# Kebii/MikuDance

Hardware: AMD Instinct MI355X
Metric: frames/sec (768x768, 16f, 20 DDIM steps) (higher is better)
Workload: dtype f16; 1 GPU; configs[1]: 768x768, 16-frame clip, 20 DDIM steps, fp16, reference_unet + denoising_unet + motion_module, CFG 3.5, one clip per GPU per step; parallelism=dp1, input_staging=rank-local (every rank stages its own clip in HBM before the timed region), reference_reuse=True, queues=1, weights=random-init SD-1.5 geometry (N(0,1/fan_in), seeds 1234/4321), width=full

## Files before the change

### include/mdance_hip.h

```cpp
#ifndef MDANCE_HIP_H
#define MDANCE_HIP_H
#include <stddef.h>
#ifdef __cplusplus
extern "C" {
#endif

#define MD_ACT_NONE 0
#define MD_ACT_SILU 1
#define MD_ACT_RELU 2
#define MD_ACT_GEGLU 3
#define MD_ACT_QUICKGELU 4

int md_version(void);
const char* md_last_error(void);

int md_gemm_f16(const void* A, int lda, const void* W, void* C, int ldc, int M, int N, int K, const void* bias,
                const void* residual, int ldr, const void* rowadd, int ldra, int rows_per_group, int act,
                int transpose_out, void* stream);

int md_conv3x3_nhwc_f16(const void* X, const void* W, void* Y, int ldy, int B, int Hin, int Win, int Cin, int Cout,
                        int stride, int upsample, const void* bias, const void* residual, int ldr,
                        const void* rowadd, int ldra, int rows_per_group, int act, void* stream);

int md_conv3x3_pad_nhwc_f16(const void* X, const void* W, void* Y, int ldy, int B, int Hin, int Win, int Cin, int Cout,
                            int stride, int upsample, int pad_lo, const void* bias, const void* residual, int ldr,
                            const void* rowadd, int ldra, int rows_per_group, int act, void* stream);

int md_conv_nhwc_f16(const void* X, int ldx, const void* W, void* Y, int ldy, int B, int Hin, int Win, int Cin, int Cout, int kw,
                     int stride, int upsample, int pad_lo, const void* bias, const void* residual, int ldr, const void* rowadd,
                     int ldra, int rows_per_group, int act, void* stream);

int md_softmax_rows_f16(void* x, int ldx, int rows, int cols, float scale, void* stream);

size_t md_groupnorm_workspace_bytes(int B, int HW, int C, int G);
int md_groupnorm_nhwc_f16(const void* x, void* y, const void* gamma, const void* beta, int B, int HW, int C, int G,
                          float eps, int silu, void* workspace, size_t ws_bytes, void* stream);

int md_groupnorm_ld_nhwc_f16(const void* x, int ldx, void* y, const void* gamma, const void* beta, int B, int HW, int C, int G,
                             float eps, int silu, void* workspace, size_t ws_bytes, void* stream);

int md_layernorm_f16(const void* x, void* y, void* y2, const void* gamma, const void* beta, const void* add, int M,
                     int C, float eps, int add_mode, int add_row_begin, int rows_per_frame, int frames, void* stream);

int md_groupnorm_plan(int B, int HW, int C, int G, int ldx, int x_align16, int table, int* threads, int* R, int* slab, int* nslab);

int md_layernorm_plan(int M, int C);

int md_gemm_ln_plan(int M, int N, int K, int act, int epi);
int md_gemm_ln_f16(const void* A, int lda, const void* Wf, const float* sc, void* C, int ldc, int M, int N, int K, float eps,
                   const void* rowadd, int ldra, int rows_per_group, int act, void* stream);

int md_groupnorm_table_f16(const void* x, int ldx, const void* gamma, const void* beta, int B, int HW, int C, int G, float eps,
                           float* table, void* workspace, size_t ws_bytes, void* stream);
int md_gemm_affine_plan(int M, int N, int K, int rows_per_image);
int md_gemm_affine_f16(const void* A, int lda, const float* table, int rows_per_image, const void* W, void* C, int ldc, int M, int N,
                       int K, const void* bias, void* stream);

int md_instnorm_spade_f16(const void* x, const void* gamma_beta, void* y, int B, int HW, int C, float eps,
                          void* stream);

int md_instnorm_spade_ld_f16(const void* x, int ldx, const void* gamma_beta, void* y, int B, int HW, int C, float eps,
                             void* stream);

int md_attention_fwd_f16(const void* Q, int ldq, const void* K, int ldk, const void* Vt, int ldvt, void* O, int ldo,
                         const int* kv_index, int B, int H, int D, int Lq, int Lk, int kv_stride, float scale,
                         void* stream);

int md_attention_plan(int D, int Lq, int Lk, int kv_stride, int ldvt, int vt_align16);

int md_temporal_attention_fwd_f16(const void* Q, int ldq, const void* K, int ldk, const void* V, int ldv, void* O,
                                  int ldo, int NB, int F, int HW, int H, int D, float scale, void* stream);

int md_temporal_attention_plan(int NB, int F, int HW, int H, int D, int aligned16, int* hg, int* pb);

int md_pack_nhwc_f16(const void* src, int src_is_f32, void* dst, int N, int F, long sB, long sF, long sC, long sY,
                     long sX, int c_begin, int c_count, int Cpad, int Ho, int Wo, int Hin, int Win, void* stream);
int md_unpack_nhwc_f16(const void* src, int ldc, void* dst, int dst_is_f32, int N, int F, long sB, long sF, long sC,
                       long sY, long sX, int C, int Ho, int Wo, void* stream);

int md_concat_channels_f16(const void* a, int Ca, const void* b, int Cb, void* out, long M, void* stream);

int md_window_accumulate(const void* pred, void* noise_sum, void* counter, const int* window, int f, int Ftot, int HW,
                         int halves, void* stream);
// ... 76 lines not shown
```

### mikudance_amd/_lib.py

```python
import ctypes
import os
from ctypes import c_char_p, c_float, c_int, c_long, c_size_t, c_void_p

_HERE = os.path.dirname(os.path.abspath(__file__))
LIB_PATH = os.path.join(_HERE, "libmdance_hip.so")

P = c_void_p
SIGNATURES = {
    "md_version": (c_int, []),
    "md_last_error": (c_char_p, []),
    "md_gemm_f16": (c_int, [P, c_int, P, P, c_int, c_int, c_int, c_int, P, P, c_int, P, c_int, c_int, c_int, c_int, P]),
    "md_conv3x3_nhwc_f16": (c_int, [P, P, P, c_int, c_int, c_int, c_int, c_int, c_int, c_int, c_int, P, P, c_int, P, c_int,
                                    c_int, c_int, P]),
    "md_conv3x3_pad_nhwc_f16": (c_int, [P, P, P, c_int, c_int, c_int, c_int, c_int, c_int, c_int, c_int, c_int, P, P, c_int, P,
                                        c_int, c_int, c_int, P]),
    "md_conv_nhwc_f16": (c_int, [P, c_int, P, P, c_int, c_int, c_int, c_int, c_int, c_int, c_int, c_int, c_int, c_int, P, P, c_int, P,
                                 c_int, c_int, c_int, P]),
    "md_set_cu_limit": (c_int, [c_int]),
    "md_gemm_plan": (c_int, [c_int, c_int, c_int, c_int, c_int, c_int, c_int]),
    "md_conv3x3_plan": (c_int, [c_int, c_int, c_int, c_int, c_int, c_int, c_int, c_int, c_int]),
    "md_gemm_plan_call": (c_int, [P, c_int, P, P, c_int, c_int, c_int, c_int, P, P, c_int, P, c_int, c_int, c_int, c_int,
                                  ctypes.POINTER(c_int), ctypes.POINTER(c_int)]),
    "md_conv_plan_call": (c_int, [P, c_int, P, P, c_int, c_int, c_int, c_int, c_int, c_int, c_int, c_int, c_int, c_int, P, P, c_int, P,
                                  c_int, c_int, c_int]),
    "md_softmax_rows_f16": (c_int, [P, c_int, c_int, c_int, c_float, P]),
    "md_groupnorm_workspace_bytes": (c_size_t, [c_int, c_int, c_int, c_int]),
    "md_groupnorm_nhwc_f16": (c_int, [P, P, P, P, c_int, c_int, c_int, c_int, c_float, c_int, P, c_size_t, P]),
    "md_groupnorm_ld_nhwc_f16": (c_int, [P, c_int, P, P, P, c_int, c_int, c_int, c_int, c_float, c_int, P, c_size_t, P]),
    "md_instnorm_spade_ld_f16": (c_int, [P, c_int, P, P, c_int, c_int, c_int, c_float, P]),
    "md_layernorm_f16": (c_int, [P, P, P, P, P, P, c_int, c_int, c_float, c_int, c_int, c_int, c_int, P]),
    "md_groupnorm_plan": (c_int, [c_int, c_int, c_int, c_int, c_int, c_int, c_int] + [ctypes.POINTER(c_int)] * 4),
    "md_layernorm_plan": (c_int, [c_int, c_int]),
    "md_gemm_ln_plan": (c_int, [c_int, c_int, c_int, c_int, c_int]),
    "md_gemm_ln_f16": (c_int, [P, c_int, P, P, P, c_int, c_int, c_int, c_int, c_float, P, c_int, c_int, c_int, P]),
    "md_groupnorm_table_f16": (c_int, [P, c_int, P, P, c_int, c_int, c_int, c_int, c_float, P, P, c_size_t, P]),
    "md_gemm_affine_plan": (c_int, [c_int, c_int, c_int, c_int]),
    "md_gemm_affine_f16": (c_int, [P, c_int, P, c_int, P, P, c_int, c_int, c_int, c_int, P, P]),
    "md_instnorm_spade_f16": (c_int, [P, P, P, c_int, c_int, c_int, c_float, P]),
    "md_attention_fwd_f16": (c_int, [P, c_int, P, c_int, P, c_int, P, c_int, P, c_int, c_int, c_int, c_int, c_int, c_int,
                                     c_float, P]),
    "md_attention_plan": (c_int, [c_int, c_int, c_int, c_int, c_int, c_int]),
    "md_temporal_attention_fwd_f16": (c_int, [P, c_int, P, c_int, P, c_int, P, c_int, c_int, c_int, c_int, c_int, c_int,
                                              c_float, P]),
    "md_temporal_attention_plan": (c_int, [c_int, c_int, c_int, c_int, c_int, c_int, ctypes.POINTER(c_int), ctypes.POINTER(c_int)]),
    "md_pack_nhwc_f16": (c_int, [P, c_int, P, c_int, c_int, c_long, c_long, c_long, c_long, c_long, c_int, c_int, c_int,
                                 c_int, c_int, c_int, c_int, P]),
    "md_unpack_nhwc_f16": (c_int, [P, c_int, P, c_int, c_int, c_int, c_long, c_long, c_long, c_long, c_long, c_int, c_int,
                                   c_int, P]),
    "md_concat_channels_f16": (c_int, [P, c_int, P, c_int, P, c_long, P]),
    "md_window_accumulate": (c_int, [P, P, P, P, c_int, c_int, c_int, c_int, P]),
    "md_window_accumulate_weighted": (c_int, [P, P, P, P, P, c_int, c_int, c_int, c_int, P]),
    "md_cfg_ddim_step": (c_int, [P, P, P, c_int, c_int, c_int, c_float, c_float, c_float, P]),
    "md_cfg_ddim_step_eta": (c_int, [P, P, P, P, c_int, c_int, c_int, c_float, c_float, c_float, c_float, P]),
    "md_cfg_multistep_step": (c_int, [P, P, P, P, P, c_int, c_int, c_int, c_float, c_float, c_float, c_float, c_float, c_float, c_float, P]),
    "md_cfg_rescale_workspace_bytes": (c_size_t, [c_int, c_int]),
    "md_cfg_guidance_rescale": (c_int, [P, P, c_int, c_int, c_int, c_float, c_float, P, c_size_t, P, P]),
    "md_cfg_ddim_step_scaled": (c_int, [P, P, P, P, P, c_int, c_int, c_int, c_float, c_float, c_float, c_float, P]),
    "md_cfg_multistep_step_scaled": (c_int, [P, P, P, P, P, P, c_int, c_int, c_int, c_float, c_float, c_float, c_float, c_float, c_float,
                                             c_float, P]),
    "md_cfg_apg_workspace_bytes": (c_size_t, [c_int, c_int]),
    "md_cfg_apg_prepare": (c_int, [P, P, P, P, c_int, c_int, c_int, c_float, c_float, c_float, c_float, c_float, P, c_size_t, P, P]),
    "md_cfg_ddim_step_apg": (c_int, [P, P, P, P, P, P, c_int, c_int, c_int, c_float, c_float, c_float, c_float, P]),
    "md_cfg_multistep_step_apg": (c_int, [P, P, P, P, P, P, P, c_int, c_int, c_int, c_float, c_float, c_float, c_float, c_float, c_float,
                                          c_float, P]),
    "md_cfg_ddim_step_pag": (c_int, [P, P, P, P, P, c_int, c_int, c_int, c_float, c_float, c_float, c_float, c_float, P]),
    "md_cfg_multistep_step_pag": (c_int, [P, P, P, P, P, P, c_int, c_int, c_int, c_float, c_float, c_float, c_float, c_float, c_float, c_float,
                                          c_float, P]),
# ... 76 lines not shown
```

### mikudance_amd/blocks.py

```python
from dataclasses import dataclass

import torch
from torch import nn

from . import ops, packing

GROUPS = 32
HEADS = 8


class _Packed(nn.Module):

    def __init__(self):
        super().__init__()
        self._pk = None

    def _apply(self, fn, *a, **k):
        self._pk = None
        return super()._apply(fn, *a, **k)

    def _load_from_state_dict(self, *a, **k):
        self._pk = None
        return super()._load_from_state_dict(*a, **k)

# ... 101 lines not shown
    def __init__(self, dim, kv_dim=None):
        super().__init__()
        self.to_q = Linear(dim, dim, bias=False)
        self.to_k = Linear(kv_dim or dim, dim, bias=False)
        self.to_v = Linear(kv_dim or dim, dim, bias=False)
        self.to_out = nn.ModuleList([Linear(dim, dim)])


class _GEGLU(nn.Module):
    def __init__(self, dim):
        super().__init__()
        self.proj = Linear(dim, dim * 8)


class FeedForward(nn.Module):

    def __init__(self, dim):
        super().__init__()
        self.net = nn.ModuleList([_GEGLU(dim), nn.Identity(), Linear(dim * 4, dim)])


def _pack_ff(ff, dev, pk, prefix="ff"):
    w, b = packing.geglu_weight(ff.net[0].proj.weight, ff.net[0].proj.bias, dev)
    pk[prefix + "1"], pk[prefix + "1b"] = w, b
    pk[prefix + "2"], pk[prefix + "2b"] = packing.linear_weight(ff.net[2].weight, dev), packing.vec(ff.net[2].bias, dev)


FUSE_NORMS = __import__("os").environ.get("MD_FUSE_NORMS", "1") != "0"


def ln_linear(pk, h, norm, lin, bias=None, rowadd=None, rows_per_group=0, act=ops.ACT_NONE, eps=1e-5):
    M, K = h.shape
    w = pk[lin]
    if FUSE_NORMS and ops.gemm_ln_plan(M, w.shape[0], K, act, rowadd is not None, a=h):
        fk = lin + ":ln"
        if fk not in pk:
            pk[fk] = packing.ln_fold(w, None if bias is None else pk[bias], pk[norm + "w"], pk[norm + "b"])
        wf, sc = pk[fk]
        return ops.gemm_ln(h, wf, sc, eps=eps, rowadd=rowadd, rows_per_group=rows_per_group, act=act)
    n = ops.layernorm(h, pk[norm + "w"], pk[norm + "b"], eps=eps)
    return ops.gemm(n, w, bias=None if bias is None else pk[bias], rowadd=rowadd, rows_per_group=rows_per_group, act=act)


def gn_linear(x, gamma, beta, eps, w, bias):
    B, C = x.shape[0], x.shape[-1]
    M = x.numel() // C
    if FUSE_NORMS and ops.gemm_affine_plan(M, w.shape[0], C, M // B, x=x):
        return ops.gemm_affine(x, ops.groupnorm_table(x, gamma, beta, GROUPS, eps), w, bias=bias)
    return ops.gemm(tokens(ops.groupnorm(x, gamma, beta, GROUPS, eps)), w, bias=bias)


def _run_ff(pk, h, norm, prefix="ff"):
    g = ln_linear(pk, h, norm, prefix + "1", bias=prefix + "1b", act=ops.ACT_GEGLU)
    return ops.gemm(g, pk[prefix + "2"], bias=pk[prefix + "2b"], residual=h)


class CrossContext:

    def __init__(self, ctx, index, lk, lpad, zero_frames=0):
        self.ctx, self.index, self.lk, self.lpad = ctx, index, lk, lpad
        self.zero_frames = zero_frames
        self.root = self
        self._slices = {}

    def rows(self, lo, hi):
        s = self._slices.get((lo, hi))
        if s is None:
            s = CrossContext(self.ctx, self.index[lo:hi].contiguous(), self.lk, self.lpad, zero_frames=max(0, min(self.zero_frames, hi) - lo))
            s.root = self.root
            self._slices[(lo, hi)] = s
        return s
# ... 290 lines not shown
```

### mikudance_amd/csrc/gemm.hip

```cpp
#include "common.h"
#include <stdlib.h>
#include <algorithm>


enum { ACT_NONE = 0, ACT_SILU = 1, ACT_RELU = 2, ACT_GEGLU = 3, ACT_QUICKGELU = 4 };

struct GemmParams {
  const half_t* A;
  const half_t* W;
  half_t* C;
  const half_t* bias;
  const half_t* residual;
  const half_t* rowadd;
  int lda, ldc, ldr, ldra;
  int M, N, K;
  int rows_per_group;
  int act;
  int transpose_out;
  int bias_rows;
  int Hin, Win, Cin, Hout, Wout, stride, upsample, pad;
  int ldx;
  int kw;
  int tiles_n, tiles_total;
  int tiles_m, group_m;
  int reverse;
};

__device__ __attribute__((aligned(64))) half_t g_zero_page[32] = {};

typedef const __attribute__((address_space(1))) void* gptr_t;
typedef __attribute__((address_space(3))) void* lptr_t;

template <int N>
__device__ __forceinline__ void wait_vmcnt() {
  asm volatile("s_waitcnt vmcnt(%0)" ::"n"(N) : "memory");
}

typedef float float2_t __attribute__((ext_vector_type(2)));
#ifdef MD_DEGRADE_GELU_TANH
__device__ __forceinline__ float md_gelu_tanh(float x) {
  const float u = 0.7978845608f * (x + 0.044715f * x * x * x);
  return 0.5f * x * (1.f + (1.f - 2.f / (__expf(2.f * u) + 1.f)));
}
#endif
__device__ __forceinline__ float2_t gelu_fast2(float2_t x) {
#ifdef MD_DEGRADE_GELU_TANH
  return float2_t{md_gelu_tanh(x.x), md_gelu_tanh(x.y)};
#endif
  const float2_t ax = {__builtin_fabsf(x.x), __builtin_fabsf(x.y)};
  float2_t p = float2_t{5.621299664e-06f, 5.621299664e-06f};
  p = p * ax + float2_t{5.105520901e-05f, 5.105520901e-05f};
  p = p * ax + float2_t{3.968613701e-05f, 3.968613701e-05f};
  p = p * ax + float2_t{3.422739239e-03f, 3.422739239e-03f};
  p = p * ax + float2_t{2.207699846e-02f, 2.207699846e-02f};
  p = p * ax + float2_t{5.207516304e-02f, 5.207516304e-02f};
  p = p * ax + float2_t{1.044273782e+00f, 1.044273782e+00f};
  p = p * p;
  p = p * p;
// ... 846 lines not shown
  plan_operands(p, epi);
  p.ldc = Cout; p.ldr = Cout; p.ldra = Cout; p.lda = Cin;
  p.Hin = Hin; p.Win = Win; p.Cin = Cin; p.stride = stride; p.upsample = upsample; p.pad = 1; p.ldx = Cin; p.kw = 3;
  p.Hout = ((Hin << upsample) + 2 - 3) / stride + 1;
  p.Wout = ((Win << upsample) + 2 - 3) / stride + 1;
  p.M = B * p.Hout * p.Wout; p.N = Cout; p.K = 9 * Cin; p.rows_per_group = p.Hout * p.Wout; p.act = ACT_NONE;
  return gemm_choose(p, true, 2, 0, ncu).k.code;
}

static int plan_call_result(const GemmParams& p, bool conv, int* blocks, int* tail_code) {
  GemmPlan plan;
  const int rc = gemm_plan_checked(p, conv, &plan);
  if (rc != MD_OK) return rc;
  if (blocks) *blocks = plan.blocks;
  if (tail_code) *tail_code = plan.tail.code;
  return plan.k.code;
}

extern "C" int md_gemm_plan_call(const void* A, int lda, const void* W, void* C, int ldc, int M, int N, int K, const void* bias, const void* residual,
                                 int ldr, const void* rowadd, int ldra, int rows_per_group, int act, int transpose_out, int* blocks,
                                 int* tail_code) {
  return plan_call_result(gemm_params(A, lda, W, C, ldc, M, N, K, bias, residual, ldr, rowadd, ldra, rows_per_group, act, transpose_out), false,
                          blocks, tail_code);
}

extern "C" int md_conv_plan_call(const void* X, int ldx, const void* W, void* Y, int ldy, int B, int Hin, int Win, int Cin, int Cout, int kw, int stride,
                                 int upsample, int pad_lo, const void* bias, const void* residual, int ldr, const void* rowadd, int ldra,
                                 int rows_per_group, int act) {
  GemmParams p;
  const int rc = conv_params(&p, X, ldx, W, Y, ldy, B, Hin, Win, Cin, Cout, kw, stride, upsample, pad_lo, bias, residual, ldr, rowadd, ldra,
                             rows_per_group, act);
  return rc != MD_OK ? rc : plan_call_result(p, true, nullptr, nullptr);
}
```

### mikudance_amd/csrc/gemm_sp.h

```cpp
#pragma once
#ifndef SP_ABL
#define SP_ABL 0
#endif

#ifdef SP_TRACE
#define SP_TRACE_N 48
__device__ unsigned long long g_sp_trace[4][SP_TRACE_N][5];
#define SP_STAMP(S)                                                                                           \
  if (!GEGLU && blockIdx.x == 0 && tr_kt < SP_TRACE_N && lane == 0)                                           \
    *reinterpret_cast<unsigned long long*>(smem + (3 * BM + 2 * BN) * 128 + ((wave * SP_TRACE_N + tr_kt) * 5 + (S)) * 8) = __builtin_readcyclecounter();
#else
#define SP_STAMP(S)
#endif

typedef unsigned uint4_t __attribute__((ext_vector_type(4)));

__device__ __attribute__((aligned(64))) half_t g_zero_cols[16384] = {};
__device__ __attribute__((aligned(64))) half_t g_sp_dump[64 * 8];

__device__ __forceinline__ float sp_acc(const floatx16& a, int r) {
  float x;
  asm volatile("v_accvgpr_read_b32 %0, %1" : "=v"(x) : "a"(a[r]));
  return x;
}

template <int MT, int NT, bool RES, bool RA>
struct SpColumn {
  half4_t b[4];
  uint4 r[RES ? MT : 1][2];
  half4_t a[RA ? MT : 1][4];
};

#ifndef SP_EPI_LA
#define SP_EPI_LA 1
#endif
template <int MT, int NT, bool CONV>
constexpr int sp_residual_lookahead() {
  constexpr int la = SP_EPI_LA < NT - 1 ? SP_EPI_LA : NT - 1;
  return CONV && MT * NT >= 15 && la > 1 ? 1 : la;
}

template <int MT, int NT, bool RES, bool RA, bool AGPR = true, bool RB = false, bool CONV = false>
__device__ __forceinline__ void sp_plain_epilogue(const GemmParams& p, const floatx16 (&acc)[MT][NT], int mw, int nw, int lc, int hi) {
  constexpr bool RA_AHEAD = RA && !RES;
  constexpr int LA = RES ? sp_residual_lookahead<MT, NT, CONV>() : 1;
  const half_t* bias = (p.bias && !RB ? p.bias : g_zero_cols) + (RB ? 0 : nw + 4 * hi);
  float rowb[MT];
  bool row_ok[MT];
  const half_t* rrow[MT];
  const half_t* arow[MT];
  half_t* crow[MT][2];
  bool crow_ok[MT][2];
#pragma unroll
  for (int i = 0; i < MT; ++i) {
    const int m = mw + i * 32 + lc;
    row_ok[i] = m < p.M;
    const int mc = row_ok[i] ? m : p.M - 1;
    rowb[i] = RB && p.bias ? (float)p.bias[mc] : 0.f;
    rrow[i] = RES ? p.residual + (size_t)mc * p.ldr + nw + 8 * hi : nullptr;
    arow[i] = RA ? p.rowadd + (size_t)(mc / p.rows_per_group) * p.ldra + nw + 4 * hi : nullptr;
#pragma unroll
    for (int h = 0; h < 2; ++h) {
      const int mr = mw + i * 32 + 16 * h + (lc & 15);
      crow_ok[i][h] = mr < p.M;
      crow[i][h] = p.C + (size_t)(crow_ok[i][h] ? mr : p.M - 1) * p.ldc + nw + 16 * ((lc >> 4) & 1) + 8 * hi;
    }
  }
  half_t* const dump = g_sp_dump + ((lc + 32 * hi) << 3);
  SpColumn<MT, NT, RES, RA> col[LA + 1];
  auto request = [&](SpColumn<MT, NT, RES, RA>& d, int j, bool ahead) {
    if constexpr (!RB) {
#pragma unroll
      for (int gi = 0; gi < 4; ++gi) d.b[gi] = *reinterpret_cast<const half4_t*>(bias + j * 32 + 8 * gi);
    }
    if constexpr (RES) {
#pragma unroll
      for (int i = 0; i < MT; ++i)
#pragma unroll
        for (int pr = 0; pr < 2; ++pr) d.r[i][pr] = *reinterpret_cast<const uint4*>(rrow[i] + j * 32 + 16 * pr);
    }
    if constexpr (RA) {
      if (ahead == RA_AHEAD) {
#pragma unroll
        for (int i = 0; i < MT; ++i)
#pragma unroll
          for (int gi = 0; gi < 4; ++gi) d.a[i][gi] = *reinterpret_cast<const half4_t*>(arow[i] + j * 32 + 8 * gi);
      }
    }
  };
#pragma unroll
  for (int j = 0; j < LA && j < NT; ++j) request(col[j % (LA + 1)], j, true);
#pragma unroll
  for (int j = 0; j < NT; ++j) {
    SpColumn<MT, NT, RES, RA>& c = col[j % (LA + 1)];
    if (j + LA < NT) request(col[(j + LA) % (LA + 1)], j + LA, true);
    if constexpr (RA && !RA_AHEAD) {
#pragma unroll
      for (int i = 0; i < MT; ++i)
#pragma unroll
        for (int gi = 0; gi < 4; ++gi) c.a[i][gi] = *reinterpret_cast<const half4_t*>(arow[i] + j * 32 + 8 * gi);
    }
    __builtin_amdgcn_sched_barrier(0);
    float bf[4][4];
#pragma unroll
    for (int gi = 0; gi < 4; ++gi)
#pragma unroll
      for (int e = 0; e < 4; ++e) bf[gi][e] = RB ? 0.f : (float)c.b[gi][e];
#pragma unroll
    for (int i = 0; i < MT; ++i) {
      unsigned rp[4][2];
      if constexpr (RES) {
#pragma unroll
        for (int pr = 0; pr < 2; ++pr) {
          const uint4 r4 = c.r[i][pr];
          const auto s0 = __builtin_amdgcn_permlane32_swap(r4.x, r4.z, false, false);
          const auto s1 = __builtin_amdgcn_permlane32_swap(r4.y, r4.w, false, false);
          rp[2 * pr][0] = s0[0]; rp[2 * pr][1] = s1[0];
          rp[2 * pr + 1][0] = s0[1]; rp[2 * pr + 1][1] = s1[1];
        }
      }
      unsigned w[4][2];
#pragma unroll
      for (int gi = 0; gi < 4; ++gi) {
        float v[4];
#pragma unroll
        for (int e = 0; e < 4; ++e) {
          v[e] = (AGPR ? sp_acc(acc[i][j], 4 * gi + e) : acc[i][j][4 * gi + e]) + (RB ? rowb[i] : bf[gi][e]);
          if constexpr (RA) v[e] += (float)c.a[i][gi][e];
        }
        if constexpr (RES) {
          half4_t rv;
          __builtin_memcpy(&rv, rp[gi], 8);
#pragma unroll
          for (int e = 0; e < 4; ++e) v[e] += (float)rv[e];
        }
        const half4_t o = {(half_t)v[0], (half_t)v[1], (half_t)v[2], (half_t)v[3]};
        __builtin_memcpy(w[gi], &o, 8);
      }
      unsigned pc[2][4];
#pragma unroll
      for (int pr = 0; pr < 2; ++pr) {
        const auto s0 = __builtin_amdgcn_permlane32_swap(w[2 * pr][0], w[2 * pr + 1][0], false, false);
        const auto s1 = __builtin_amdgcn_permlane32_swap(w[2 * pr][1], w[2 * pr + 1][1], false, false);
        pc[pr][0] = s0[0]; pc[pr][1] = s1[0]; pc[pr][2] = s0[1]; pc[pr][3] = s1[1];
      }
      unsigned lo[4], hi4[4];
#pragma unroll
      for (int d = 0; d < 4; ++d) {
        const auto t = __builtin_amdgcn_permlane16_swap(pc[0][d], pc[1][d], false, false);
        lo[d] = t[0]; hi4[d] = t[1];
      }
#pragma unroll
      for (int h = 0; h < 2; ++h) {
        const uint4 v4 = h ? uint4{hi4[0], hi4[1], hi4[2], hi4[3]} : uint4{lo[0], lo[1], lo[2], lo[3]};
        if (SP_ABL & 64) asm volatile("" ::"v"(v4.x), "v"(v4.y), "v"(v4.z), "v"(v4.w));
        else *reinterpret_cast<uint4*>(crow_ok[i][h] ? crow[i][h] + j * 32 : dump) = v4;
      }
      __builtin_amdgcn_sched_barrier(0);
    }
  }
}

template <bool CONV, bool GEGLU, int MT, int NT, bool RESM = false>
__global__ __launch_bounds__(256, 1) void gemm_sp_kernel(GemmParams p) {
#if defined(__HIP_DEVICE_COMPILE__)
  constexpr int BK = 64;
  constexpr int BM = 64 * MT, BN = 64 * NT;
  constexpr int ROWB = BK * 2, RPI = 1024 / ROWB;
  constexpr int PA = BM / RPI / 4, PB = BN / RPI / 4;
  static_assert(PA + PB == 16 || PA + PB == 14 || PA + PB == 12 || PA + PB == 10, "issue schedule");
  constexpr int NP0 = PA + PB == 10 ? 3 : (PA + PB == 12 ? 4 : 6), NP1 = PA + PB == 10 ? 3 : 4, NP2 = (PA + PB - NP0 - NP1) / 2, NP3 = NP2;
  static_assert(NP0 + NP1 + NP2 + NP3 == PA + PB && PB >= NP0, "issue schedule");
  static_assert(!GEGLU || NT % 2 == 0, "GEGLU pairs 32-column sub-tiles (2q, 2q+1) of a wave");
  constexpr int ASZ = BM * ROWB, WSZ = BN * ROWB, WBASE = 3 * ASZ;
  extern __shared__ __attribute__((aligned(16))) char smem[];

  const int tid = threadIdx.x;
  const int lane = tid & 63;
  const int wave = __builtin_amdgcn_readfirstlane(tid >> 6);
  const int wm = wave >> 1, wn = wave & 1;
  const int lrow = lane >> 3, pslot = lane & 7;
  const int nk = p.K / BK;
  const int nwg = p.tiles_total;
  const int ntile = (nwg - (int)blockIdx.x + (int)gridDim.x - 1) / (int)gridDim.x;

  auto tile_origin = [&](int i, int& m0, int& n0) {
    const int v = (int)blockIdx.x + i * (int)gridDim.x;
    const int q = nwg >> 3, r = nwg & 7, xcd = v & 7, idx = v >> 3;
    int t = (xcd < r ? xcd * (q + 1) : r * (q + 1) + (xcd - r) * q) + idx;
    if (p.reverse) t = nwg - 1 - t;
    const int gsz = p.group_m * p.tiles_n;
    const int grp = t / gsz, first = grp * p.group_m;
    const int rows = min(p.group_m, p.tiles_m - first);
    const int l = t - grp * gsz;
    const int tn = l / rows;
    m0 = (first + l - tn * rows) * BM;
    n0 = tn * BN;
// ... 293 lines not shown
            gelu_fast2_x<8>(gl);
            __builtin_amdgcn_sched_barrier(0);
            unsigned w[4][2];
#pragma unroll
            for (int c = 0; c < 8; ++c) {
              const float2_t hv = (float2_t{sp_acc(acc[i][2 * q], 2 * c), sp_acc(acc[i][2 * q], 2 * c + 1)} + bh[c]) * gl[c];
              typedef _Float16 h2_t __attribute__((ext_vector_type(2)));
              const h2_t o = {(half_t)hv.x, (half_t)hv.y};
              __builtin_memcpy(&w[c >> 1][c & 1], &o, 4);
            }
            unsigned pc[2][4];
#pragma unroll
            for (int pr = 0; pr < 2; ++pr) {
              const auto s0 = __builtin_amdgcn_permlane32_swap(w[2 * pr][0], w[2 * pr + 1][0], false, false);
              const auto s1 = __builtin_amdgcn_permlane32_swap(w[2 * pr][1], w[2 * pr + 1][1], false, false);
              pc[pr][0] = s0[0]; pc[pr][1] = s1[0]; pc[pr][2] = s0[1]; pc[pr][3] = s1[1];
            }
            uint4 vv[2];
            {
              const auto t0 = __builtin_amdgcn_permlane16_swap(pc[0][0], pc[1][0], false, false);
              const auto t1 = __builtin_amdgcn_permlane16_swap(pc[0][1], pc[1][1], false, false);
              const auto t2 = __builtin_amdgcn_permlane16_swap(pc[0][2], pc[1][2], false, false);
              const auto t3 = __builtin_amdgcn_permlane16_swap(pc[0][3], pc[1][3], false, false);
              vv[0] = uint4{t0[0], t1[0], t2[0], t3[0]};
              vv[1] = uint4{t0[1], t1[1], t2[1], t3[1]};
            }
#pragma unroll
            for (int h = 0; h < 2; ++h) *reinterpret_cast<uint4*>(drow[h]) = vv[h];
            __builtin_amdgcn_sched_barrier(0);
          }
        }
      } else {
        const int mw = m0 + wm * (32 * MT), nw = n0 + wn * (32 * NT);
        if constexpr (RESM) {
          if (p.rowadd) sp_plain_epilogue<MT, NT, false, true>(p, acc, mw, nw, lc, hi);
          else sp_plain_epilogue<MT, NT, false, false>(p, acc, mw, nw, lc, hi);
        } else if (p.bias_rows) sp_plain_epilogue<MT, NT, false, false, true, true>(p, acc, mw, nw, lc, hi);
        else if (p.residual && p.rowadd && !(SP_ABL & 32)) sp_plain_epilogue<MT, NT, true, true, true, false, CONV>(p, acc, mw, nw, lc, hi);
        else if (p.residual && !(SP_ABL & 32)) sp_plain_epilogue<MT, NT, true, false, true, false, CONV>(p, acc, mw, nw, lc, hi);
        else if (p.rowadd) sp_plain_epilogue<MT, NT, false, true>(p, acc, mw, nw, lc, hi);
        else sp_plain_epilogue<MT, NT, false, false>(p, acc, mw, nw, lc, hi);
      }
    }
  }
  wait_vmcnt<0>();
#ifdef SP_TRACE
  if (!GEGLU && blockIdx.x == 0) {
    __syncthreads();
    for (int i = tid; i < 4 * SP_TRACE_N * 5; i += 256)
      (&g_sp_trace[0][0][0])[i] = *reinterpret_cast<const unsigned long long*>(smem + (3 * BM + 2 * BN) * 128 + i * 8);
  }
#endif
#undef SP_TRACE_NEXT
#undef SP_BODY
#undef SP_STEP
#undef SP_RES_MULT
#undef SP_RES_ISSUE
#endif
}

template <bool CONV, bool GEGLU, int NT>
static bool sp_eligible(const GemmParams& p) {
  constexpr int BN = 64 * NT;
  if (p.transpose_out || p.N % BN != 0 || p.K % 64 != 0 || p.K < 128 || (p.N > 16384 && !p.bias_rows)) return false;
  if (p.bias_rows && (p.residual || p.rowadd || CONV || GEGLU)) return false;
  if (!GEGLU && p.act != ACT_NONE) return false;
  if (CONV && p.Cin % 64 != 0) return false;
// ... 3 lines not shown
  if (!al16(p.C) || p.ldc % 8 != 0) return false;
  if (p.bias && !p.bias_rows && !al16(p.bias)) return false;
  if (p.residual && (!al16(p.residual) || p.ldr % 8 != 0)) return false;
  if (p.rowadd && (!al16(p.rowadd) || p.ldra % 8 != 0)) return false;
  return true;
}

template <int MT, int NT>
static bool sp_resm(const GemmParams& p) {
  static const int resm = md_env_int("MD_SP_RESM", 1);
  return resm && p.residual && !p.bias_rows && !(SP_ABL & 32) && p.K / 64 >= MT * NT + 1 &&
         ((unsigned long long)(p.M - 1) * p.ldr + p.N) * 2 < (1ull << 31);
}

template <bool CONV, bool GEGLU, int NT, int MT>
static void launch_sp(GemmParams& p, bool resm, int ncu, hipStream_t stream) {
  constexpr int BM = 64 * MT, BN = 64 * NT;
#ifdef SP_TRACE
  constexpr size_t smem = (size_t)(3 * BM + 2 * BN) * 128 + (GEGLU ? 0 : 4 * SP_TRACE_N * 5 * 8);
  static_assert(smem <= 160 * 1024, "trace build: the stamps live behind the ring");
#else
  constexpr size_t smem = (size_t)(3 * BM + 2 * BN) * 128;
#endif
  md_ensure_dynamic_lds<gemm_sp_kernel<CONV, GEGLU, MT, NT>>((int)smem);
  constexpr int group_m = 8;
  p.tiles_n = p.N / BN;
  p.tiles_m = cdiv(p.M, BM);
  p.tiles_total = p.tiles_m * p.tiles_n;
  p.group_m = group_m;
  static const int rev = md_env_int("MD_SP_REVERSE", 1);
  const bool big_a = (size_t)p.M * (size_t)p.lda * 2 > ((size_t)256 << 20);
  p.reverse = !CONV && !GEGLU && !p.bias_rows && big_a && (rev == 2 || (rev == 1 && p.K >= 4 * p.N));
  const int grid = p.tiles_total < ncu ? p.tiles_total : ncu;
  if constexpr (!GEGLU) {
    if (resm) {
      md_ensure_dynamic_lds<gemm_sp_kernel<CONV, false, MT, NT, true>>((int)smem);
      hipLaunchKernelGGL((gemm_sp_kernel<CONV, false, MT, NT, true>), dim3(grid), dim3(256), smem, stream, p);
      return;
    }
  }
  hipLaunchKernelGGL((gemm_sp_kernel<CONV, GEGLU, MT, NT>), dim3(grid), dim3(256), smem, stream, p);
}

#ifdef SP_TRACE
extern "C" int md_debug_sp_trace(void* dst) {
  return (int)hipMemcpyFromSymbol(dst, HIP_SYMBOL(g_sp_trace), sizeof(unsigned long long) * 4 * SP_TRACE_N * 5);
}
#endif
```

### mikudance_amd/csrc/norm.hip

```cpp
#include "common.h"
#ifndef GN_UNROLL
#define GN_UNROLL 4
#endif
#ifndef GN_THREADS
#define GN_THREADS 512
#endif
template <typename T>
__device__ __forceinline__ void norm_store(T* p, const T& v) { *p = v; }
#ifndef GN_SLAB
#define GN_SLAB 32
#endif

__device__ __forceinline__ float med3(float a, float b, float c) { return fmaxf(fminf(a, b), fminf(fmaxf(a, b), c)); }
__device__ __forceinline__ float gn_pilot(const half_t* __restrict__ ximg, int HW, int ldx, int g, int cpg) {
  const half_t* p = ximg + g * cpg;
  return med3((float)p[0], (float)p[(size_t)(HW >> 1) * ldx + (cpg >> 1)], (float)p[(size_t)(HW - 1) * ldx + cpg - 1]);
}
__global__ void gn_stats_kernel(const half_t* __restrict__ x, float* __restrict__ part, float* __restrict__ pilot, int HW, int C, int ldx, int G, int R,
                                int slab, int nslab) {
  extern __shared__ float sh[];
  const int cch = C >> 3;
  const int cc = threadIdx.x % cch, r = threadIdx.x / cch;
  const int b = blockIdx.y, sl = blockIdx.x;
  const int p0 = sl * slab, p1 = min(p0 + slab, HW);
// ... 573 lines not shown
  if (C == 320) return 720;
#endif
  return 700 + (C <= 512 ? 1 : C <= 1024 ? 2 : C <= 1536 ? 3 : 4);
}

extern "C" int md_layernorm_plan(int M, int C) { return ln_plan(M, C); }

extern "C" int md_layernorm_f16(const void* x, void* y, void* y2, const void* gamma, const void* beta, const void* add, int M, int C, float eps,
                                int add_mode, int add_row_begin, int rows_per_frame, int frames, void* stream) {
  const int code = ln_plan(M, C);
  if (code < 0) return code;
  MD_CHECK_ARG(add_mode == 0 || (add != nullptr && y2 != nullptr), "md_layernorm: add_mode needs add and y2");
  MD_CHECK_ARG(add_mode != 2 || (rows_per_frame > 0 && frames > 0), "md_layernorm: add_mode 2 needs rows_per_frame and frames");
  const dim3 grid(cdiv(M, 4 * LN_R)), block(256);
  hipStream_t st = (hipStream_t)stream;
  if (code == 720) {
    hipLaunchKernelGGL(layernorm320_kernel, dim3(cdiv(M, 32)), block, 0, st, (const half_t*)x, (half_t*)y, (half_t*)y2, (const half_t*)gamma,
                       (const half_t*)beta, (const half_t*)add, M, eps, add_mode, add_row_begin, rows_per_frame, frames);
    MD_CHECK_LAUNCH("md_layernorm");
    return MD_OK;
  }
#define LN_LAUNCH(MC)                                                                                                                          \
  hipLaunchKernelGGL(layernorm_kernel<MC>, grid, block, 0, st, (const half_t*)x, (half_t*)y, (half_t*)y2, (const half_t*)gamma, (const half_t*)beta, \
                     (const half_t*)add, M, C, eps, add_mode, add_row_begin, rows_per_frame, frames)
  if (code == 701) LN_LAUNCH(1);
  else if (code == 702) LN_LAUNCH(2);
  else if (code == 703) LN_LAUNCH(3);
  else LN_LAUNCH(4);
#undef LN_LAUNCH
  MD_CHECK_LAUNCH("md_layernorm");
  return MD_OK;
}

__global__ __launch_bounds__(256) void instnorm_spade_kernel(const half_t* __restrict__ x, const half_t* __restrict__ gb, half_t* __restrict__ y, int HW,
                                                             int C, int ldx, float eps) {
  __shared__ float ss[32][64], sq[32][64], mean_s[64], rstd_s[64];
  const int cc = threadIdx.x & 7, r = threadIdx.x >> 3;
  const int b = blockIdx.y, c0 = blockIdx.x * 64 + cc * 8;
  const half_t* xb = x + (size_t)b * HW * ldx + c0;
  const half8_t ka = *reinterpret_cast<const half8_t*>(xb), kb = *reinterpret_cast<const half8_t*>(xb + (size_t)(HW >> 1) * ldx),
                kc = *reinterpret_cast<const half8_t*>(xb + (size_t)(HW - 1) * ldx);
  float k8[8];
#pragma unroll
  for (int e = 0; e < 8; ++e) k8[e] = med3((float)ka[e], (float)kb[e], (float)kc[e]);
  float s[8], q[8];
#pragma unroll
  for (int e = 0; e < 8; ++e) s[e] = q[e] = 0.f;
  for (int p = r; p < HW; p += 32) {
    const half8_t v = *reinterpret_cast<const half8_t*>(xb + (size_t)p * ldx);
#pragma unroll
    for (int e = 0; e < 8; ++e) {
      const float f = (float)v[e] - k8[e];
      s[e] += f;
      q[e] += f * f;
    }
  }
#pragma unroll
  for (int e = 0; e < 8; ++e) {
    ss[r][cc * 8 + e] = s[e];
    sq[r][cc * 8 + e] = q[e];
  }
  __syncthreads();
  if (threadIdx.x < 64) {
    float a = 0.f, c2 = 0.f;
    for (int rr = 0; rr < 32; ++rr) {
      a += ss[rr][threadIdx.x];
// ... 81 lines not shown
```

### mikudance_amd/ops.py

```python
import ctypes

import torch

from . import _lib

ACT_NONE, ACT_SILU, ACT_RELU, ACT_GEGLU, ACT_QUICKGELU = 0, 1, 2, 3, 4
F16 = torch.float16


def _st():
    return torch.cuda.current_stream().cuda_stream


def _p(t):
    return 0 if t is None else t.data_ptr()


def _chk(t, name, dtype=F16):
    if t is None:
        return
    if not t.is_cuda:
        raise _lib.MdanceHipError(f"{name} must live on the GPU: mikudance_amd has no CPU path")
    if t.dtype != dtype:
        raise _lib.MdanceHipError(f"{name} must be {dtype}, got {t.dtype}")
# ... 92 lines not shown
                    2.0 * B * Ho * Wo * cout * 3 * kw * Cin, 2.0 * (B * H * W * Cin + cout * 3 * kw * Cin + B * Ho * Wo * cout)))
    return out


def conv_plan(x, w, cout, bias=None, residual=None, rowadd=None, rows_per_group=0, act=ACT_NONE, stride=1, upsample=False,
              out=None, pad_lo=1, kw=3):
    args, _, _ = _conv_args(x, w, cout, bias, residual, rowadd, rows_per_group, act, stride, upsample, out, pad_lo, kw)
    return _lib.load().md_conv_plan_call(*args)


def _dense16(t):
    return t is None or (t.data_ptr() % 16 == 0 and t.stride(-2) % 8 == 0 and t.stride(-1) == 1)


def gemm_ln_plan(M, N, K, act=ACT_NONE, rowadd=False, a=None):
    return _dense16(a) and bool(_lib.load().md_gemm_ln_plan(M, N, K, act, 2 if rowadd else 0))


def gemm_ln(a, wf, sc, eps=1e-5, rowadd=None, rows_per_group=0, act=ACT_NONE, out=None):
    lda = _rowmajor(a, "a")
    _chk(wf, "wf"); _chk(sc, "sc", torch.float32); _chk(rowadd, "rowadd")
    M, K = a.shape
    N = wf.shape[0]
    assert wf.shape[1] == K and wf.is_contiguous() and sc.shape == (2, N) and sc.is_contiguous(), (wf.shape, sc.shape, K)
    if out is None:
        out = torch.empty((M, N // 2 if act == ACT_GEGLU else N), device=a.device, dtype=F16)
    ldc = _rowmajor(out, "out")
    ldra = _rowmajor(rowadd, "rowadd") if rowadd is not None else 0
    if rowadd is not None and (rows_per_group <= 0 or rowadd.shape[0] * rows_per_group < M or rowadd.shape[1] < N):
        raise _lib.MdanceHipError(f"gemm_ln: row term {tuple(rowadd.shape)} does not cover M={M} rows in groups of {rows_per_group} x N={N}")
    _lib.call("md_gemm_ln_f16", a.data_ptr(), lda, wf.data_ptr(), sc.data_ptr(), out.data_ptr(), ldc, M, N, K, float(eps), _p(rowadd), ldra,
              rows_per_group, act, _st(),
              meta=(f"gemm M={M} N={N} K={K}" + (" geglu" if act == ACT_GEGLU else "") + " ln", 2.0 * M * N * K, 2.0 * (M * K + N * K + M * N)))
    return out


_workspaces = {}


def _workspace(who, device, need, dtype=torch.float32, floor=0):
    cache = _workspaces.setdefault(who, {})
    key = (device, torch.cuda.current_stream().cuda_stream)
    ws = cache.get(key)
    if ws is None or ws.numel() * dtype.itemsize < need:
        ws = cache[key] = torch.empty((max(need, floor) + dtype.itemsize - 1) // dtype.itemsize, device=device, dtype=dtype)
    return ws


def _gn_workspace(x, B, HW, C, groups):
    return _workspace("groupnorm", x.device, _lib.load().md_groupnorm_workspace_bytes(B, HW, C, groups), floor=1 << 20)


def gemm_affine_plan(M, N, K, rows_per_image, x=None):
    return _dense16(x) and bool(_lib.load().md_gemm_affine_plan(M, N, K, rows_per_image))


def groupnorm_table(x, gamma, beta, groups, eps):
    _chk(gamma, "gamma"); _chk(beta, "beta")
    ldx = _pixel_pitch(x, "x")
    B, C = x.shape[0], x.shape[-1]
    HW = x.numel() // (B * C)
    ws = _gn_workspace(x, B, HW, C, groups)
    table = torch.empty((B, 2, C), device=x.device, dtype=torch.float32)
    _lib.call("md_groupnorm_table_f16", x.data_ptr(), ldx, gamma.data_ptr(), beta.data_ptr(), B, HW, C, groups, float(eps), table.data_ptr(),
              ws.data_ptr(), ws.numel() * 4, _st(), meta=(f"groupnorm B={B} HW={HW} C={C} stats", 0.0, 2.0 * B * HW * C))
    return table
# ... 379 lines not shown
```

Baseline: 7.351 frames/s.

## Fold LayerNorm into GEMM epilogue via precomputed row stats kernel

After: 7.368 frames/s, median of 3. Within noise of the previous version (+0.2%).

```diff
diff --git a/include/mdance_hip.h b/include/mdance_hip.h
--- a/include/mdance_hip.h
+++ b/include/mdance_hip.h
@@ -49,6 +49,12 @@
 int md_gemm_ln_plan(int M, int N, int K, int act, int epi);
 int md_gemm_ln_f16(const void* A, int lda, const void* Wf, const float* sc, void* C, int ldc, int M, int N, int K, float eps,
                    const void* rowadd, int ldra, int rows_per_group, int act, void* stream);
+
+int md_row_stats_plan(int M, int C, int ldx, int x_align16);
+int md_row_stats_f16(const void* x, int ldx, float* stats, int M, int C, float eps, void* stream);
+int md_gemm_ln_stats_plan(int M, int N, int K, int act, int epi);
+int md_gemm_ln_stats_f16(const void* A, int lda, const void* Wf, const float* sc, const float* stats, void* C, int ldc, int M, int N,
+                         int K, const void* rowadd, int ldra, int rows_per_group, int act, void* stream);
 
 int md_groupnorm_table_f16(const void* x, int ldx, const void* gamma, const void* beta, int B, int HW, int C, int G, float eps,
                            float* table, void* workspace, size_t ws_bytes, void* stream);
diff --git a/mikudance_amd/_lib.py b/mikudance_amd/_lib.py
--- a/mikudance_amd/_lib.py
+++ b/mikudance_amd/_lib.py
@@ -33,6 +33,10 @@
     "md_layernorm_plan": (c_int, [c_int, c_int]),
     "md_gemm_ln_plan": (c_int, [c_int, c_int, c_int, c_int, c_int]),
     "md_gemm_ln_f16": (c_int, [P, c_int, P, P, P, c_int, c_int, c_int, c_int, c_float, P, c_int, c_int, c_int, P]),
+    "md_row_stats_plan": (c_int, [c_int, c_int, c_int, c_int]),
+    "md_row_stats_f16": (c_int, [P, c_int, P, c_int, c_int, c_float, P]),
+    "md_gemm_ln_stats_plan": (c_int, [c_int, c_int, c_int, c_int, c_int]),
+    "md_gemm_ln_stats_f16": (c_int, [P, c_int, P, P, P, P, c_int, c_int, c_int, c_int, P, c_int, c_int, c_int, P]),
     "md_groupnorm_table_f16": (c_int, [P, c_int, P, P, c_int, c_int, c_int, c_int, c_float, P, P, c_size_t, P]),
     "md_gemm_affine_plan": (c_int, [c_int, c_int, c_int, c_int]),
     "md_gemm_affine_f16": (c_int, [P, c_int, P, c_int, P, P, c_int, c_int, c_int, c_int, P, P]),
diff --git a/mikudance_amd/blocks.py b/mikudance_amd/blocks.py
--- a/mikudance_amd/blocks.py
+++ b/mikudance_amd/blocks.py
@@ -157,11 +157,15 @@
 def ln_linear(pk, h, norm, lin, bias=None, rowadd=None, rows_per_group=0, act=ops.ACT_NONE, eps=1e-5):
     M, K = h.shape
     w = pk[lin]
-    if FUSE_NORMS and ops.gemm_ln_plan(M, w.shape[0], K, act, rowadd is not None, a=h):
+    fused = FUSE_NORMS and ops.gemm_ln_plan(M, w.shape[0], K, act, rowadd is not None, a=h)
+    swept = FUSE_NORMS and not fused and ops.gemm_ln_stats_plan(M, w.shape[0], K, act, rowadd is not None, a=h)
+    if fused or swept:
         fk = lin + ":ln"
         if fk not in pk:
             pk[fk] = packing.ln_fold(w, None if bias is None else pk[bias], pk[norm + "w"], pk[norm + "b"])
         wf, sc = pk[fk]
+        if swept:
+            return ops.gemm_ln_stats(h, wf, sc, ops.row_stats(h, eps=eps), rowadd=rowadd, rows_per_group=rows_per_group, act=act)
         return ops.gemm_ln(h, wf, sc, eps=eps, rowadd=rowadd, rows_per_group=rows_per_group, act=act)
     n = ops.layernorm(h, pk[norm + "w"], pk[norm + "b"], eps=eps)
     return ops.gemm(n, w, bias=None if bias is None else pk[bias], rowadd=rowadd, rows_per_group=rows_per_group, act=act)
diff --git a/mikudance_amd/csrc/gemm.hip b/mikudance_amd/csrc/gemm.hip
--- a/mikudance_amd/csrc/gemm.hip
+++ b/mikudance_amd/csrc/gemm.hip
@@ -24,6 +24,8 @@
   int tiles_n, tiles_total;
   int tiles_m, group_m;
   int reverse;
+  const float* lnst;
+  const float* lnsc;
 };
 
 __device__ __attribute__((aligned(64))) half_t g_zero_page[32] = {};
@@ -936,3 +938,40 @@
                              rows_per_group, act);
   return rc != MD_OK ? rc : plan_call_result(p, true, nullptr, nullptr);
 }
+
+static int ln_stats_classes() {
+  static const int m = md_env_int("MD_LN_STATS", 3);
+  return m;
+}
+
+static int ln_stats_code(const GemmPlan& plan, const GemmParams& p) {
+  if (p.act != ACT_NONE || p.residual || p.transpose_out || p.K < 640) return 0;
+  if (plan.blocks != 1 || !plan.k.tile || plan.k.swapped || plan.k.resm) return 0;
+  return 3000 + plan.k.tile->code;
+}
+
+extern "C" int md_gemm_ln_stats_plan(int M, int N, int K, int act, int epi) {
+  if (M <= 0 || N <= 0 || K <= 0 || K % 64 || (epi & 1)) return 0;
+  if (!(ln_stats_classes() & ((epi & 2) ? 2 : 1))) return 0;
+  GemmParams p = {};
+  plan_operands(p, epi & 2);
+  p.M = M; p.N = N; p.K = K; p.lda = K; p.ldc = N; p.ldra = N; p.rows_per_group = M; p.act = act;
+  int sp, force_nt;
+  gemm_knobs(&sp, &force_nt);
+  return ln_stats_code(gemm_choose(p, false, sp, force_nt, md_device_cus()), p);
+}
+
+extern "C" int md_gemm_ln_stats_f16(const void* A, int lda, const void* Wf, const float* sc, const float* stats, void* C, int ldc, int M, int N, int K,
+                                    const void* rowadd, int ldra, int rows_per_group, int act, void* stream) {
+  GemmParams p = gemm_params(A, lda, Wf, C, ldc, M, N, K, nullptr, nullptr, 0, rowadd, ldra, rows_per_group, act, 0);
+  GemmPlan plan;
+  if (const int rc = gemm_plan_checked(p, false, &plan)) return rc;
+  MD_CHECK_ARG(ln_stats_code(plan, p) != 0, "md_gemm_ln_stats: no row-affine kernel for M=%d N=%d K=%d act=%d (ask md_gemm_ln_stats_plan first)", M, N, K, act);
+  MD_CHECK_ARG(sc != nullptr && al16(sc) && stats != nullptr && (reinterpret_cast<uintptr_t>(stats) & 7) == 0,
+               "md_gemm_ln_stats: sc must be 16-byte aligned, stats 8-byte aligned");
+  MD_CHECK_ARG((const void*)stats != C && A != C, "md_gemm_ln_stats: in place is not supported");
+  p.lnst = stats; p.lnsc = sc;
+  gemm_launch(plan, p, (hipStream_t)stream);
+  MD_CHECK_LAUNCH("md_gemm_ln_stats");
+  return MD_OK;
+}
diff --git a/mikudance_amd/csrc/gemm_sp.h b/mikudance_amd/csrc/gemm_sp.h
--- a/mikudance_amd/csrc/gemm_sp.h
+++ b/mikudance_amd/csrc/gemm_sp.h
@@ -24,9 +24,10 @@
   return x;
 }
 
-template <int MT, int NT, bool RES, bool RA>
+template <int MT, int NT, bool RES, bool RA, bool LNS = false>
 struct SpColumn {
   half4_t b[4];
+  floatx4 s[LNS ? 4 : 1], c[LNS ? 4 : 1];
   uint4 r[RES ? MT : 1][2];
   half4_t a[RA ? MT : 1][4];
 };
@@ -40,11 +41,14 @@
   return CONV && MT * NT >= 15 && la > 1 ? 1 : la;
 }
 
-template <int MT, int NT, bool RES, bool RA, bool AGPR = true, bool RB = false, bool CONV = false>
+template <int MT, int NT, bool RES, bool RA, bool AGPR = true, bool RB = false, bool CONV = false, bool LNS = false>
 __device__ __forceinline__ void sp_plain_epilogue(const GemmParams& p, const floatx16 (&acc)[MT][NT], int mw, int nw, int lc, int hi) {
+  static_assert(!LNS || (!RES && !RB && !CONV), "the row-affine flavour: plain GEMM, no residual, column operands");
   constexpr bool RA_AHEAD = RA && !RES;
   constexpr int LA = RES ? sp_residual_lookahead<MT, NT, CONV>() : 1;
   const half_t* bias = (p.bias && !RB ? p.bias : g_zero_cols) + (RB ? 0 : nw + 4 * hi);
+  [[maybe_unused]] const float* lns = LNS ? p.lnsc + nw + 4 * hi : nullptr;
+  [[maybe_unused]] float2_t rt[MT];
   float rowb[MT];
   bool row_ok[MT];
   const half_t* rrow[MT];
@@ -57,6 +61,7 @@
     row_ok[i] = m < p.M;
     const int mc = row_ok[i] ? m : p.M - 1;
     rowb[i] = RB && p.bias ? (float)p.bias[mc] : 0.f;
+    if constexpr (LNS) rt[i] = *reinterpret_cast<const float2_t*>(p.lnst + 2 * (size_t)mc);
     rrow[i] = RES ? p.residual + (size_t)mc * p.ldr + nw + 8 * hi : nullptr;
     arow[i] = RA ? p.rowadd + (size_t)(mc / p.rows_per_group) * p.ldra + nw + 4 * hi : nullptr;
 #pragma unroll
@@ -67,9 +72,15 @@
     }
   }
   half_t* const dump = g_sp_dump + ((lc + 32 * hi) << 3);
-  SpColumn<MT, NT, RES, RA> col[LA + 1];
-  auto request = [&](SpColumn<MT, NT, RES, RA>& d, int j, bool ahead) {
-    if constexpr (!RB) {
+  SpColumn<MT, NT, RES, RA, LNS> col[LA + 1];
+  auto request = [&](SpColumn<MT, NT, RES, RA, LNS>& d, int j, bool ahead) {
+    if constexpr (LNS) {
+#pragma unroll
+      for (int gi = 0; gi < 4; ++gi) {
+        d.s[gi] = *reinterpret_cast<const floatx4*>(lns + j * 32 + 8 * gi);
+        d.c[gi] = *reinterpret_cast<const floatx4*>(lns + p.N + j * 32 + 8 * gi);
+      }
+    } else if constexpr (!RB) {
 #pragma unroll
       for (int gi = 0; gi < 4; ++gi) d.b[gi] = *reinterpret_cast<const half4_t*>(bias + j * 32 + 8 * gi);
     }
@@ -92,7 +103,7 @@
   for (int j = 0; j < LA && j < NT; ++j) request(col[j % (LA + 1)], j, true);
 #pragma unroll
   for (int j = 0; j < NT; ++j) {
-    SpColumn<MT, NT, RES, RA>& c = col[j % (LA + 1)];
+    SpColumn<MT, NT, RES, RA, LNS>& c = col[j % (LA + 1)];
     if (j + LA < NT) request(col[(j + LA) % (LA + 1)], j + LA, true);
     if constexpr (RA && !RA_AHEAD) {
 #pragma unroll
@@ -105,7 +116,7 @@
 #pragma unroll
     for (int gi = 0; gi < 4; ++gi)
 #pragma unroll
-      for (int e = 0; e < 4; ++e) bf[gi][e] = RB ? 0.f : (float)c.b[gi][e];
+      for (int e = 0; e < 4; ++e) bf[gi][e] = RB || LNS ? 0.f : (float)c.b[gi][e];
 #pragma unroll
     for (int i = 0; i < MT; ++i) {
       unsigned rp[4][2];
@@ -125,7 +136,9 @@
         float v[4];
 #pragma unroll
         for (int e = 0; e < 4; ++e) {
-          v[e] = (AGPR ? sp_acc(acc[i][j], 4 * gi + e) : acc[i][j][4 * gi + e]) + (RB ? rowb[i] : bf[gi][e]);
+          const float a = AGPR ? sp_acc(acc[i][j], 4 * gi + e) : acc[i][j][4 * gi + e];
+          if constexpr (LNS) v[e] = __builtin_fmaf(rt[i].x, a, __builtin_fmaf(rt[i].y, c.s[gi][e], c.c[gi][e]));
+          else v[e] = a + (RB ? rowb[i] : bf[gi][e]);
           if constexpr (RA) v[e] += (float)c.a[i][gi][e];
         }
         if constexpr (RES) {
@@ -161,8 +174,9 @@
   }
 }
 
-template <bool CONV, bool GEGLU, int MT, int NT, bool RESM = false>
+template <bool CONV, bool GEGLU, int MT, int NT, bool RESM = false, bool LNS = false>
 __global__ __launch_bounds__(256, 1) void gemm_sp_kernel(GemmParams p) {
+  static_assert(!LNS || (!CONV && !GEGLU && !RESM), "the row-affine (folded LayerNorm) epilogue: plain GEMMs without a residual");
 #if defined(__HIP_DEVICE_COMPILE__)
   constexpr int BK = 64;
   constexpr int BM = 64 * MT, BN = 64 * NT;
@@ -522,7 +536,10 @@
         }
       } else {
         const int mw = m0 + wm * (32 * MT), nw = n0 + wn * (32 * NT);
-        if constexpr (RESM) {
+        if constexpr (LNS) {
+          if (p.rowadd) sp_plain_epilogue<MT, NT, false, true, true, false, false, true>(p, acc, mw, nw, lc, hi);
+          else sp_plain_epilogue<MT, NT, false, false, true, false, false, true>(p, acc, mw, nw, lc, hi);
+        } else if constexpr (RESM) {
           if (p.rowadd) sp_plain_epilogue<MT, NT, false, true>(p, acc, mw, nw, lc, hi);
           else sp_plain_epilogue<MT, NT, false, false>(p, acc, mw, nw, lc, hi);
         } else if (p.bias_rows) sp_plain_epilogue<MT, NT, false, false, true, true>(p, acc, mw, nw, lc, hi);
@@ -592,6 +609,13 @@
   const bool big_a = (size_t)p.M * (size_t)p.lda * 2 > ((size_t)256 << 20);
   p.reverse = !CONV && !GEGLU && !p.bias_rows && big_a && (rev == 2 || (rev == 1 && p.K >= 4 * p.N));
   const int grid = p.tiles_total < ncu ? p.tiles_total : ncu;
+  if constexpr (!GEGLU && !CONV) {
+    if (p.lnst) {
+      md_ensure_dynamic_lds<gemm_sp_kernel<false, false, MT, NT, false, true>>((int)smem);
+      hipLaunchKernelGGL((gemm_sp_kernel<false, false, MT, NT, false, true>), dim3(grid), dim3(256), smem, stream, p);
+      return;
+    }
+  }
   if constexpr (!GEGLU) {
     if (resm) {
       md_ensure_dynamic_lds<gemm_sp_kernel<CONV, false, MT, NT, true>>((int)smem);
diff --git a/mikudance_amd/csrc/norm.hip b/mikudance_amd/csrc/norm.hip
--- a/mikudance_amd/csrc/norm.hip
+++ b/mikudance_amd/csrc/norm.hip
@@ -629,6 +629,92 @@
   return MD_OK;
 }
 
+template <int MAXC>
+__global__ __launch_bounds__(256) void row_stats_kernel(const half_t* __restrict__ x, float* __restrict__ stats, int M, int C, int ldx, float eps) {
+  typedef float f2 __attribute__((ext_vector_type(2)));
+  const int lane = threadIdx.x & 63;
+  const int row0 = (blockIdx.x * 4 + (threadIdx.x >> 6)) * LN_R;
+  if (row0 >= M) return;
+  const int cch = C >> 3;
+  float v[LN_R][MAXC][8];
+#pragma unroll
+  for (int r = 0; r < LN_R; ++r) {
+    const int row = min(row0 + r, M - 1);
+#pragma unroll
+    for (int k = 0; k < MAXC; ++k) {
+      const int c = lane + k * 64;
+      half8_t h = {0, 0, 0, 0, 0, 0, 0, 0};
+      if (c < cch) h = *reinterpret_cast<const half8_t*>(x + (size_t)row * ldx + c * 8);
+#pragma unroll
+      for (int e = 0; e < 8; ++e) v[r][k][e] = (float)h[e];
+    }
+  }
+  float mu[LN_R], sq[LN_R];
+#pragma unroll
+  for (int r = 0; r < LN_R; ++r) {
+    float sum = 0.f;
+#pragma unroll
+    for (int k = 0; k < MAXC; ++k)
+#pragma unroll
+      for (int e = 0; e < 8; ++e) sum += v[r][k][e];
+    mu[r] = sum;
+  }
+#pragma unroll
+  for (int o = 32; o > 0; o >>= 1)
+#pragma unroll
+    for (int r = 0; r < LN_R; ++r) mu[r] += __shfl_xor(mu[r], o, 64);
+#pragma unroll
+  for (int r = 0; r < LN_R; ++r) {
+    mu[r] /= (float)C;
+    float s = 0.f;
+#pragma unroll
+    for (int k = 0; k < MAXC; ++k) {
+      if (lane + k * 64 < cch) {
+#pragma unroll
+        for (int e = 0; e < 8; ++e) {
+          const float d = v[r][k][e] - mu[r];
+          s += d * d;
+        }
+      }
+    }
+    sq[r] = s;
+  }
+#pragma unroll
+  for (int o = 32; o > 0; o >>= 1)
+#pragma unroll
+    for (int r = 0; r < LN_R; ++r) sq[r] += __shfl_xor(sq[r], o, 64);
+#pragma unroll
+  for (int r = 0; r < LN_R; ++r) {
+    const float rs = rsqrtf(sq[r] / (float)C + eps);
+    if (lane == r && row0 + r < M) *reinterpret_cast<f2*>(stats + (size_t)(row0 + r) * 2) = f2{rs, -mu[r] * rs};
+  }
+}
+
+static int row_stats_plan(int M, int C, int ldx, bool x16) {
+  MD_CHECK_ARG(M > 0 && C > 0 && C % 8 == 0 && C <= 8 * 64 * LN_MAXC, "md_row_stats: M=%d must be positive, C=%d a multiple of 8 and <= %d", M, C, 8 * 64 * LN_MAXC);
+  MD_CHECK_ARG(ldx >= C && ldx % 8 == 0 && x16, "md_row_stats: ldx=%d must be a multiple of 8 and >= C=%d, x 16-byte aligned", ldx, C);
+  return 730 + (C <= 512 ? 1 : C <= 1024 ? 2 : C <= 1536 ? 3 : 4);
+}
+
+extern "C" int md_row_stats_plan(int M, int C, int ldx, int x_align16) { return row_stats_plan(M, C, ldx, x_align16 != 0); }
+
+extern "C" int md_row_stats_f16(const void* x, int ldx, float* stats, int M, int C, float eps, void* stream) {
+  const int code = row_stats_plan(M, C, ldx, (reinterpret_cast<uintptr_t>(x) & 15) == 0);
+  if (code < 0) return code;
+  MD_CHECK_ARG(stats != nullptr && (reinterpret_cast<uintptr_t>(stats) & 7) == 0, "md_row_stats: stats must be 8-byte aligned");
+  MD_CHECK_ARG(eps > 0.f && eps <= 3.0e38f, "md_row_stats: eps=%g must be positive and finite (a constant row has variance 0)", (double)eps);
+  const dim3 grid(cdiv(M, 4 * LN_R)), block(256);
+  hipStream_t st = (hipStream_t)stream;
+#define RS_LAUNCH(MC) hipLaunchKernelGGL(row_stats_kernel<MC>, grid, block, 0, st, (const half_t*)x, stats, M, C, ldx, eps)
+  if (code == 731) RS_LAUNCH(1);
+  else if (code == 732) RS_LAUNCH(2);
+  else if (code == 733) RS_LAUNCH(3);
+  else RS_LAUNCH(4);
+#undef RS_LAUNCH
+  MD_CHECK_LAUNCH("md_row_stats");
+  return MD_OK;
+}
+
 __global__ __launch_bounds__(256) void instnorm_spade_kernel(const half_t* __restrict__ x, const half_t* __restrict__ gb, half_t* __restrict__ y, int HW,
                                                              int C, int ldx, float eps) {
   __shared__ float ss[32][64], sq[32][64], mean_s[64], rstd_s[64];
diff --git a/mikudance_amd/ops.py b/mikudance_amd/ops.py
--- a/mikudance_amd/ops.py
+++ b/mikudance_amd/ops.py
@@ -148,6 +148,41 @@
     _lib.call("md_gemm_ln_f16", a.data_ptr(), lda, wf.data_ptr(), sc.data_ptr(), out.data_ptr(), ldc, M, N, K, float(eps), _p(rowadd), ldra,
               rows_per_group, act, _st(),
               meta=(f"gemm M={M} N={N} K={K}" + (" geglu" if act == ACT_GEGLU else "") + " ln", 2.0 * M * N * K, 2.0 * (M * K + N * K + M * N)))
+    return out
+
+
+def gemm_ln_stats_plan(M, N, K, act=ACT_NONE, rowadd=False, a=None):
+    return _lib.load().md_gemm_ln_stats_plan(M, N, K, act, 2 if rowadd else 0) if _dense16(a) else 0
+
+
+def row_stats(x, eps=1e-5, out=None):
+    ldx = _rowmajor(x, "x")
+    M, C = x.shape
+    if out is None:
+        out = torch.empty((M, 2), device=x.device, dtype=torch.float32)
+    _chk(out, "out", torch.float32)
+    assert out.shape == (M, 2) and out.is_contiguous()
+    _lib.call("md_row_stats_f16", x.data_ptr(), ldx, out.data_ptr(), M, C, float(eps), _st(),
+              meta=(f"layernorm M={M} C={C} stats", 0.0, 2.0 * M * C + 8.0 * M))
+    return out
+
+
+def gemm_ln_stats(a, wf, sc, stats, rowadd=None, rows_per_group=0, act=ACT_NONE, out=None):
+    lda = _rowmajor(a, "a")
+    _chk(wf, "wf"); _chk(sc, "sc", torch.float32); _chk(stats, "stats", torch.float32); _chk(rowadd, "rowadd")
+    M, K = a.shape
+    N = wf.shape[0]
+    assert wf.shape[1] == K and wf.is_contiguous() and sc.shape == (2, N) and sc.is_contiguous(), (wf.shape, sc.shape, K)
+    assert stats.shape == (M, 2) and stats.is_contiguous(), stats.shape
+    if out is None:
+        out = torch.empty((M, N), device=a.device, dtype=F16)
+    ldc = _rowmajor(out, "out")
+    ldra = _rowmajor(rowadd, "rowadd") if rowadd is not None else 0
+    if rowadd is not None and (rows_per_group <= 0 or rowadd.shape[0] * rows_per_group < M or rowadd.shape[1] < N):
+        raise _lib.MdanceHipError(f"gemm_ln_stats: row term {tuple(rowadd.shape)} does not cover M={M} rows in groups of {rows_per_group} x N={N}")
+    _lib.call("md_gemm_ln_stats_f16", a.data_ptr(), lda, wf.data_ptr(), sc.data_ptr(), stats.data_ptr(), out.data_ptr(), ldc, M, N, K,
+              _p(rowadd), ldra, rows_per_group, act, _st(),
+              meta=(f"gemm M={M} N={N} K={K} lnstats", 2.0 * M * N * K, 2.0 * (M * K + N * K + M * N)))
     return out
 
 
```
